# sohmandal/classpose

Measured on AMD Instinct MI355X. Metric: wsi_tiles_per_sec, higher is better.
Workload: dtype bf16; 1 GPU; configs[1]: synthetic 10000x10000 WSI (1936 tiles), tile 256 / overlap 32, conic 7 classes, ViT-L ClassTransformer depth 24 random-init, batch 32 sub-tiles = 8 WSI tiles/step, every step a distinct batch of the rank's shard (tiles sharded k % n_gpus, at most 256 distinct batches resident, longer runs wrap) streamed pinned host -> hipMemcpyAsync inside the timed region (the reader decodes ahead int; slide=10000, tile=256, overlap=32, batch_subtiles=32, distinct_batches=145, records_gathered=2048, decode_ahead_batches_at_t0=4, device_resident_batches_at_t0=1

## Files before the change

classpose_amd/_lib.py:

```python
from __future__ import annotations

import ctypes as C
import os
import subprocess

_HERE = os.path.dirname(os.path.abspath(__file__))
LIB_PATH = os.path.join(_HERE, "libclasspose_hip.so")
DEBUG_LIB_PATH = os.path.join(_HERE, "libclasspose_hip_debug.so")
CSRC = os.path.join(_HERE, "csrc")

ABI_VERSION = 3
DT_BF16, DT_F16, DT_F32 = 0, 1, 2
DTYPE_CODE = {"bf16": DT_BF16, "fp16": DT_F16, "fp32": DT_F32}
PROF_KINDS = ("fc1", "attention", "qkv", "proj", "fc2", "patch_embed", "neck_head")
FC1_KERNEL_NAME = "k_gemm4w<GELU + folded LayerNorm, one wave per SIMD> = void k_gemm4w<1, 0, false>(Gemm4wArgs)"


class CpxTiling(C.Structure):
    _fields_ = [("H", C.c_int), ("W", C.c_int), ("ypad1", C.c_int), ("xpad1", C.c_int),
                ("Ly", C.c_int), ("Lx", C.c_int), ("ny", C.c_int), ("nx", C.c_int),
                ("bsize", C.c_int), ("augment", C.c_int),
                ("ystart", C.c_int * 16), ("xstart", C.c_int * 16)]


# ... 128 lines not shown
    "cpx_stain_samples_workspace_bytes": (_sz, [_i, C.c_longlong]),
    "cpx_stain_samples": (_i, [_p, _p, _p, _i, C.c_longlong, _p, _d, _p, C.c_longlong, _p, _p, _p, _p, _sz, _p]),
    "cpx_he_stain_u8": (_i, [_p, _i, _i, _i, _p, _p, _p, _p, _p]),
    "cpx_warp_affine_pool_stain_u8": (_i, [_p, _p, _p, _p, _i, C.c_longlong, _p, _p, _i, _p, _p, _i, _p, _p, _p, _i, _i, _i, _p, _p,
                                           _p, _p]),
    "cpx_find_contours_ccomp_host": (_i, [_p, _i, _i, _p, _i, _p, _p, _p, _i]),
    "cpx_polygonize_workspace_bytes": (_sz, [_i, _i, _i, _i]),
    "cpx_polygonize_device": (_i, [_p, _p, _p, _i, _i, _i, _i, _d, _p, _p, _i, _p, _p, _p, _p]),
    "cpx_polygonize_host": (_i, [_p, _i, _i, _p, _i, _d, _d, _d, _p, _i, _p]),
    "cpx_dedup_pairs_workspace_bytes": (_sz, [_i, _i, _i]),
    "cpx_dedup_pairs": (_i, [_p, _i, _d, _d, _d, _i, _i, _d, _p, C.c_longlong, _p, _p, _sz, _p]),
    "cpx_write_geojson": (_i, [C.c_char_p, C.c_char_p, _p, C.c_int64, _p, _p, _p, _p, C.c_int64, _p, _i, _d, _d, _i]),
}
_PRIVATE = {
    "cpx_gemm_set_variant": (None, [_i]),
    "cpx_attention_set_variant": (None, [_i]),
    "cpx_gemm_set_nt": (None, [_i]),
    "cpx_follow_set_early_exit": (None, [_i]),
    "cpx_follow_set_lds_window": (None, [_i]),
    "cpx_gemm_set_reverse": (None, [_i]),
    "cpx_attention_set_xcd_order": (None, [_i]),
    "cpx_gemm_set_big": (None, [_i]),
    "cpx_gemm_set_persistent": (None, [_i]),
    "cpx_gemm_set_persistent_qkv": (None, [_i]),
    "cpx_postproc_set_fused": (None, [_i]),
    "cpx_gemm_set_direct": (None, [_i]),
    "cpx_gemm4w": (_i, [_p, _p, _i, _i, _i, _p, _p, _i, _p]),
    "cpx_gemm4w_set_variant": (None, [_i]),
    "cpx_gemm_set_4w": (None, [_i]),
    "cpx_net_set_mlp_parts": (None, [_i]),
    "cpx_gemm_set_balanced": (None, [_i]),
    "cpx_gemm_set_l2_block": (None, [_i]),
    "cpx_gemm_ln_dt": (_i, [_i, _p, _p, _i, _i, _i, _i, _p, _p, _p, _i, _p, _p, _p, _p]),
    "cpx_row_stats_dt": (_i, [_i, _p, _i, _p, _p]),
    "cpx_im2col3_f32_debug": (_i, [_p, _i, _p, _p]),
    "cpx_unet_head_layout": (_i, [C.POINTER(CpxConvOp), _i, _i, _i, C.POINTER(_sz), C.POINTER(_i)]),
}

_lib = None


class CpxError(RuntimeError):
    pass


def build(force: bool = False) -> str:
    if force:
# ... 98 lines not shown
```

classpose_amd/csrc/cpx_gemm.hip:

```cpp
#include "cpx_internal.h"
#include <type_traits>

typedef __attribute__((ext_vector_type(8))) __bf16 bf16x8;
typedef __attribute__((ext_vector_type(8))) _Float16 f16x8;
typedef __attribute__((ext_vector_type(4))) float f32x4;

#define BM 128
#define BN 128
#define BK 64
#define GEMM_THREADS 256
#define TILE_BYTES (128 * 128)
#define STAGE_BYTES (2 * TILE_BYTES)

template <bool NT_POSSIBLE, bool WT_POSSIBLE = false>
__device__ __forceinline__ void st16(void *p, uint4 v, bool nt, bool wt = false) {
    if (WT_POSSIBLE && wt) {
        typedef unsigned u32x4_t __attribute__((ext_vector_type(4)));
        u32x4_t w = {v.x, v.y, v.z, v.w};
        if (NT_POSSIBLE && nt) asm volatile("global_store_dwordx4 %0, %1, off sc1 nt" ::"v"(p), "v"(w) : "memory");
        else asm volatile("global_store_dwordx4 %0, %1, off sc1" ::"v"(p), "v"(w) : "memory");
    } else if (NT_POSSIBLE && nt) {
        typedef unsigned u32x4_t __attribute__((ext_vector_type(4)));
        u32x4_t w = {v.x, v.y, v.z, v.w};
        __builtin_nontemporal_store(w, reinterpret_cast<u32x4_t *>(p));
    } else {
        *reinterpret_cast<uint4 *>(p) = v;
    }
}
struct GemmArgs {
    const unsigned short *A;
    const unsigned short *W;
    int M, N, K;
    const float *bias;
    const void *aux;
    void *out;
    int ld_out;
    int tiles_n, n_blocks;
    int l2_block;
    int rev_m;
    int nt_out;
    const float *ln_stats;
    const float *ln_colsum;
    float *stats_out;
// ... 248 lines not shown
__device__ __forceinline__ void g2_read_x(u32x4 (&fx)[4][2], unsigned b0, unsigned b1) {
    fx[0][0] = lds_read128<HM * G2_HALF + 0 * 2048>(b0); fx[0][1] = lds_read128<HM * G2_HALF + 0 * 2048>(b1);
    fx[1][0] = lds_read128<HM * G2_HALF + 1 * 2048>(b0); fx[1][1] = lds_read128<HM * G2_HALF + 1 * 2048>(b1);
    fx[2][0] = lds_read128<HM * G2_HALF + 2 * 2048>(b0); fx[2][1] = lds_read128<HM * G2_HALF + 2 * 2048>(b1);
    fx[3][0] = lds_read128<HM * G2_HALF + 3 * 2048>(b0); fx[3][1] = lds_read128<HM * G2_HALF + 3 * 2048>(b1);
}
template <int HN>
__device__ __forceinline__ void g2_read_w(u32x4 (&fw)[2][2], unsigned b0, unsigned b1) {
    fw[0][0] = lds_read128<(2 + HN) * G2_HALF + 0 * 2048>(b0); fw[0][1] = lds_read128<(2 + HN) * G2_HALF + 0 * 2048>(b1);
    fw[1][0] = lds_read128<(2 + HN) * G2_HALF + 1 * 2048>(b0); fw[1][1] = lds_read128<(2 + HN) * G2_HALF + 1 * 2048>(b1);
}
template <bool F16, bool FIRST = false>
__device__ __forceinline__ void g2_mma(f32x4 (&acc)[4][2], const u32x4 (&fx)[4][2], const u32x4 (&fw)[2][2]) {
    __builtin_amdgcn_s_setprio(1);
#pragma unroll
    for (int ks = 0; ks < 2; ++ks)
#pragma unroll
        for (int mb = 0; mb < 4; ++mb)
#pragma unroll
            for (int nb = 0; nb < 2; ++nb)
                acc[mb][nb] = mfma16v<F16>(fw[nb][ks], fx[mb][ks], (FIRST && ks == 0) ? (f32x4){0.f, 0.f, 0.f, 0.f} : acc[mb][nb]);
    __builtin_amdgcn_s_setprio(0);
}
#define G2_BAR() __builtin_amdgcn_s_barrier()
#define G2_LGKM0() do { asm volatile("s_waitcnt lgkmcnt(0)" ::: "memory"); __builtin_amdgcn_sched_barrier(0); } while (0)

#define G2F_LN 1
#define G2F_STATS 2
#define G2F_BAL 64
#define G2F_DIRECT 32
template <int EPI, bool F16, int FLAGS>
__global__ void __launch_bounds__(G2_THREADS, 2) k_gemm256(GemmArgs g) {
    constexpr bool LN_IN = (FLAGS & G2F_LN) != 0 && EPI != CPX_EPI_RESID_BF16 && EPI != CPX_EPI_POS_BF16;
    constexpr bool STATS = (FLAGS & G2F_STATS) != 0 && (EPI == CPX_EPI_RESID_BF16 || EPI == CPX_EPI_POS_BF16);
    extern __shared__ __attribute__((aligned(16))) char smem[];
    const int tid = threadIdx.x, lane = tid & 63;
    const int wave = __builtin_amdgcn_readfirstlane(tid >> 6);
    const int wm = wave >> 2, wn = wave & 3;
    const int fr = lane & 15, fq = lane >> 4;
    int bid = blockIdx.x;
    {
        const int nxcd = 8, q = g.n_blocks / nxcd, r = g.n_blocks % nxcd, x = bid % nxcd;
        bid = (x < r ? x * (q + 1) : r * (q + 1) + (x - r) * q) + bid / nxcd;
    }
    int tile_m, tile_n;
    {
// ... 226 lines not shown
                if (c16 == 16)
                    *reinterpret_cast<float2 *>(g.stats_out + ((size_t)(m0 + ml) * LN_SLOTS + tile_n) * 2) = make_float2(sm, sq);
            }
        }
    }
}


#define G2P_STG_OFF G2_BUF
#define G2P_TAIL G2_LN_OFF
#define G2P_LDS_BYTES (G2_LN_OFF + 4096)
template <int EPI, bool F16, int FLAGS>
__global__ void __launch_bounds__(G2_THREADS, 2) k_gemm256p(GemmArgs g) {
    constexpr bool LN_IN = (FLAGS & G2F_LN) != 0 && EPI != CPX_EPI_RESID_BF16;
    constexpr bool STATS = (FLAGS & G2F_STATS) != 0 && EPI == CPX_EPI_RESID_BF16;
    extern __shared__ __attribute__((aligned(16))) char smem[];
    const int wave = __builtin_amdgcn_readfirstlane((int)threadIdx.x >> 6);
    const int wm = wave >> 2, wn = wave & 3;
    const int K = g.K, nk = K / 64, nblk = g.n_blocks, tiles_m = g.n_blocks / g.tiles_n;
    auto coords = [&](int v, int &m0_, int &n0_, int &tn_) {
        const int nxcd = 8, q = nblk / nxcd, r = nblk % nxcd, x = v % nxcd;
        int bid = (x < r ? x * (q + 1) : r * (q + 1) + (x - r) * q) + v / nxcd;
        int tile_m, tile_n;
        if (EPI == CPX_EPI_QKV_BF16 && g.l2_block == 3) {
            const int x = v & 7, slot = (v >> 3) & 31, i = v >> 8, rx = tiles_m >> 3, full = rx >> 4;
            int rg, cg;
            if (i < 6 * full) {
                const int rnd = i / 6, j = i - rnd * 6;
                rg = 2 * rnd + (j < 4 ? j >> 1 : j - 4); cg = j < 4 ? j & 1 : 2;
            } else {
                const int j = i - 6 * full;
                rg = 2 * full; cg = j < 2 ? j : 2;
            }
            tile_m = x * rx + rg * 8 + (slot >> 2);
            tile_n = cg * 4 + (slot & 3);
        } else if (g.l2_block && (tiles_m & 7) == 0 && (g.tiles_n & 3) == 0) {
            const int grp = bid >> 5, w_ = bid & 31, cgn = g.tiles_n >> 2, rgn = tiles_m >> 3;
            const int rg = g.l2_block == 2 ? grp % rgn : grp / cgn, cg = g.l2_block == 2 ? grp / rgn : grp - rg * cgn;
            tile_m = rg * 8 + (w_ >> 2);
            tile_n = cg * 4 + (w_ & 3);
        } else {
            tile_m = bid / g.tiles_n;
            tile_n = bid - tile_m * g.tiles_n;
        }
        if (g.rev_m) tile_m = tiles_m - 1 - tile_m;
        m0_ = tile_m * 256; n0_ = tile_n * 256; tn_ = tile_n;
    };
    char *sdst = smem + wave * 1024;
    const __amdgpu_buffer_rsrc_t rsrcX = __builtin_amdgcn_make_buffer_rsrc((void *)g.A, 0, 0x7FFFFFFF, 0x00020000);
    const __amdgpu_buffer_rsrc_t rsrcW = __builtin_amdgcn_make_buffer_rsrc((void *)g.W, 0, 0x7FFFFFFF, 0x00020000);
    const unsigned k64b = (unsigned)K * 128u, k128b = (unsigned)K * 256u;
    auto stage_at = [&](unsigned voff, unsigned sX, unsigned sW, int which, int t) {
        const unsigned so = (which < 2 ? sX : sW) + (which & 1) * k128b + (unsigned)t * 128u;
        char *d = sdst + (t & 1) * G2_BUF + which * G2_HALF;
        if (which < 2) {
            __builtin_amdgcn_raw_ptr_buffer_load_lds(rsrcX, (__attribute__((address_space(3))) void *)d, 16, voff, so, 0, 0);
            __builtin_amdgcn_raw_ptr_buffer_load_lds(rsrcX, (__attribute__((address_space(3))) void *)(d + 8192), 16, voff, so + k64b, 0, 0);
        } else {
            __builtin_amdgcn_raw_ptr_buffer_load_lds(rsrcW, (__attribute__((address_space(3))) void *)d, 16, voff, so, 0, 0);
            __builtin_amdgcn_raw_ptr_buffer_load_lds(rsrcW, (__attribute__((address_space(3))) void *)(d + 8192), 16, voff, so + k64b, 0, 0);
        }
    };
    const unsigned lds0 = (unsigned)(size_t)(__attribute__((address_space(3))) char *)smem;
    int v = blockIdx.x, m0, n0, tile_n;
    coords(v, m0, n0, tile_n);
    bool prefetched = false;
    for (;;) {
        const int vn = v + (int)gridDim.x;
        const bool has_next = vn < nblk;
        int m0n = 0, n0n = 0, tile_nn = 0;
        if (has_next) coords(vn, m0n, n0n, tile_nn);
        int tid = threadIdx.x;
        asm volatile("" : "+v"(tid));
        const int lane = tid & 63, fr = lane & 15, fq = lane >> 4, c16 = tid & 31;
        const int srow = tid >> 3, kc = (tid & 7) ^ (srow & 7);
        unsigned xb[2][2], wb[2][2];
#pragma unroll
        for (int ks = 0; ks < 2; ++ks) {
            const unsigned sw = (unsigned)(((ks * 4 + fq) ^ (fr & 7)) << 4);
            xb[0][ks] = lds0 + (wm * 64 + fr) * 128 + sw;
            wb[0][ks] = lds0 + (wn * 32 + fr) * 128 + sw;
            xb[1][ks] = xb[0][ks] + G2_BUF;
            wb[1][ks] = wb[0][ks] + G2_BUF;
        }
        const unsigned voff = ((unsigned)srow * (unsigned)K + (unsigned)kc * 8u) * 2u;
        const unsigned sX = (unsigned)m0 * (unsigned)K * 2u, sW = (unsigned)n0 * (unsigned)K * 2u;
        auto stage = [&](int which, int t) { stage_at(voff, sX, sW, which, t); };
        float4 st_a = make_float4(0.f, 0.f, 0.f, 0.f), st_b = st_a;
        float bias_v = 0.f, csum_v = 0.f;
        if (tid < 256) {
            if (LN_IN) {
                st_a = *reinterpret_cast<const float4 *>(g.ln_stats + (size_t)(m0 + tid) * 8);
                st_b = *reinterpret_cast<const float4 *>(g.ln_stats + (size_t)(m0 + tid) * 8 + 4);
            }
        } else {
            if (g.bias) bias_v = g.bias[n0 + tid - 256];
            if (LN_IN) csum_v = g.ln_colsum[n0 + tid - 256];
        }
        auto park_tile_vectors = [&]() {
            if (tid < 256) {
                if (LN_IN) {
                    const float inv_k = 1.0f / K;
                    const float sum = (st_a.x + st_a.z) + (st_b.x + st_b.z), sq = (st_a.y + st_a.w) + (st_b.y + st_b.w);
                    const float mean = sum * inv_k;
                    const float rstd = rsqrtf(fmaxf(sq * inv_k - mean * mean, 0.f) + 1e-6f);
                    *reinterpret_cast<float2 *>(smem + G2P_TAIL + tid * 8) = make_float2(rstd, -mean * rstd);
                }
            } else {
                *reinterpret_cast<float *>(smem + G2P_TAIL + 2048 + (tid - 256) * 4) = bias_v;
                *reinterpret_cast<float *>(smem + G2P_TAIL + 3072 + (tid - 256) * 4) = csum_v;
            }
        };
        constexpr bool BAL = (FLAGS & G2F_BAL) != 0;
        if (prefetched) {
            park_tile_vectors();
            if (nk > 1) { stage(0, 1); stage(3, 1); if constexpr (BAL) stage(2, 1); }
        } else {
            stage(0, 0); stage(2, 0); stage(3, 0); stage(1, 0);
            if (nk > 1) { stage(0, 1); stage(3, 1); if constexpr (BAL) stage(2, 1); }
            park_tile_vectors();
        }
        asm volatile("s_waitcnt lgkmcnt(0)" ::: "memory");
        if constexpr (BAL) asm volatile("s_waitcnt vmcnt(6)" ::: "memory");
        else if (nk > 1) asm volatile("s_waitcnt vmcnt(4)" ::: "memory");
        else asm volatile("s_waitcnt vmcnt(0)" ::: "memory");
        G2_BAR();
        f32x4 acc[2][2][4][2];
        u32x4 fx[4][2], fw[2][2], fw2[2][2];
        if constexpr (BAL) g2_read_w<0>(fw, wb[0][0], wb[0][1]);
// ... 62 lines not shown
        if constexpr (BAL) {
            G2_TILE_BAL(0, 0, true, 0, fw, fw2)
            G2_TILE_BAL(1, 1, false, 2, fw2, fw)
            for (int t = 2; t + 2 < nk; t += 2) {
                G2_TILE_BAL(t, 0, false, 2, fw, fw2)
                G2_TILE_BAL(t + 1, 1, false, 2, fw2, fw)
            }
            G2_TILE_BAL(nk - 2, 0, false, 3, fw, fw2)
            G2_TILE_BAL(nk - 1, 1, false, 4, fw2, fw)
        } else {
        G2_TILE_PLAIN(0, 0, true, -1)
        G2_TILE_PLAIN(1, 1, false, -1)
        for (int t = 2; t < nk; t += 2) {
            G2_TILE_PLAIN(t, 0, false, -1)
            G2_TILE_PLAIN(t + 1, 1, false, -1)
        }
        }
#undef G2_TILE_BAL
#undef G2_VM
#undef G2_TILE_PLAIN
        if (wm == 0) G2_BAR();
        __builtin_amdgcn_sched_barrier(0);

        const bool vt_tile = (EPI == CPX_EPI_QKV_BF16) && n0 >= 2048;
        bool next_issued = false;
        const unsigned sXn = (unsigned)m0n * (unsigned)K * 2u, sWn = (unsigned)n0n * (unsigned)K * 2u;
        auto prefetch_next = [&]() {
            stage_at(voff, sXn, sWn, 0, 0); stage_at(voff, sXn, sWn, 2, 0); stage_at(voff, sXn, sWn, 3, 0); stage_at(voff, sXn, sWn, 1, 0);
            next_issued = true;
        };
        if (vt_tile) {
#pragma unroll
            for (int hm = 0; hm < 2; ++hm)
#pragma unroll
                for (int hn = 0; hn < 2; ++hn)
#pragma unroll
                    for (int mb = 0; mb < 4; ++mb)
#pragma unroll
                        for (int nb = 0; nb < 2; ++nb) {
                            const int ml = hm * 128 + wm * 64 + mb * 16 + fr;
                            const int nl = hn * 128 + wn * 32 + nb * 16 + fq * 4;
                            f32x4 vv = acc[hm][hn][mb][nb];
                            const float4 b = *reinterpret_cast<const float4 *>(smem + G2P_TAIL + 2048 + nl * 4);
                            if constexpr (LN_IN) {
                                const float4 cs = *reinterpret_cast<const float4 *>(smem + G2P_TAIL + 3072 + nl * 4);
                                const float2 pr = *reinterpret_cast<const float2 *>(smem + G2P_TAIL + ml * 8);
                                vv[0] = fmaf(vv[0], pr.x, fmaf(pr.y, cs.x, b.x)); vv[1] = fmaf(vv[1], pr.x, fmaf(pr.y, cs.y, b.y));
                                vv[2] = fmaf(vv[2], pr.x, fmaf(pr.y, cs.z, b.z)); vv[3] = fmaf(vv[3], pr.x, fmaf(pr.y, cs.w, b.w));
                            } else {
                                vv[0] += b.x; vv[1] += b.y; vv[2] += b.z; vv[3] += b.w;
                            }
                            const unsigned p01 = pack2<F16>(vv[0], vv[1]), p23 = pack2<F16>(vv[2], vv[3]);
                            *reinterpret_cast<unsigned short *>(smem + (nl + 0) * G2_EPI_LD + ml * 2) = (unsigned short)p01;
                            *reinterpret_cast<unsigned short *>(smem + (nl + 1) * G2_EPI_LD + ml * 2) = (unsigned short)(p01 >> 16);
                            *reinterpret_cast<unsigned short *>(smem + (nl + 2) * G2_EPI_LD + ml * 2) = (unsigned short)p23;
                            *reinterpret_cast<unsigned short *>(smem + (nl + 3) * G2_EPI_LD + ml * 2) = (unsigned short)(p23 >> 16);
                        }
            asm volatile("s_waitcnt lgkmcnt(0)" ::: "memory");
            G2_BAR();
            unsigned short *vT = (unsigned short *)g.aux;
            const size_t s_ = (size_t)(m0 >> 10), t0 = (size_t)(m0 & 1023);
#pragma unroll 4
            for (int it = 0; it < 16; ++it) {
                const int row = it * 16 + (tid >> 5);
                const int c = n0 - 2048 + row;
                uint4 vv = *reinterpret_cast<const uint4 *>(smem + row * G2_EPI_LD + c16 * 16);
                st16<EPI == CPX_EPI_QKV_BF16, EPI == CPX_EPI_QKV_BF16>(vT + ((s_ * 16 + (c >> 6)) * 64 + (c & 63)) * 1024 + t0 + c16 * 8, vv, (g.nt_out & 4) != 0, (g.nt_out & 16) != 0);
            }
            asm volatile("s_waitcnt lgkmcnt(0)" ::: "memory");
            G2_BAR();
        } else if constexpr (EPI != CPX_EPI_RESID_BF16 && (FLAGS & G2F_DIRECT) != 0) {
            if (has_next) prefetch_next();
            const __amdgpu_buffer_rsrc_t rsrcO = __builtin_amdgcn_make_buffer_rsrc((void *)g.out, 0, 0x7FFFFFFF, 0x00020000);
            const unsigned ldb = (unsigned)g.ld_out * 2u;
            const unsigned ovoff = (unsigned)(wm * 64 + fr) * ldb + (unsigned)(wn * 32 + ((fq & 1) << 4) + ((fq >> 1) << 3)) * 2u;
            const unsigned so0 = (unsigned)m0 * ldb + (unsigned)n0 * 2u;
#pragma unroll
            for (int hm = 0; hm < 2; ++hm) {
                float ln_rs[4], ln_nm[4];
                if constexpr (LN_IN) {
#pragma unroll
                    for (int mb = 0; mb < 4; ++mb) {
                        const float2 pr = *reinterpret_cast<const float2 *>(smem + G2P_TAIL + (hm * 128 + wm * 64 + mb * 16 + fr) * 8);
                        ln_rs[mb] = pr.x; ln_nm[mb] = pr.y;
                    }
                }
#pragma unroll
                for (int hn = 0; hn < 2; ++hn) {
                    float4 b[2], cs[2];
#pragma unroll
                    for (int nb = 0; nb < 2; ++nb) {
                        const int nl = hn * 128 + wn * 32 + nb * 16 + fq * 4;
                        b[nb] = *reinterpret_cast<const float4 *>(smem + G2P_TAIL + 2048 + nl * 4);
                        cs[nb] = make_float4(0.f, 0.f, 0.f, 0.f);
// ... 11 lines not shown
                                vv[2] = fmaf(vv[2], rs, fmaf(nm, cs[nb].z, b[nb].z)); vv[3] = fmaf(vv[3], rs, fmaf(nm, cs[nb].w, b[nb].w));
                            } else {
                                vv[0] += b[nb].x; vv[1] += b[nb].y; vv[2] += b[nb].z; vv[3] += b[nb].w;
                            }
                            if constexpr (EPI == CPX_EPI_GELU_BF16) {
#pragma unroll
                                for (int r = 0; r < 4; ++r) vv[r] = gelu_erf(vv[r]);
                            } else if constexpr (EPI == CPX_EPI_RELU_BF16) {
#pragma unroll
                                for (int r = 0; r < 4; ++r) vv[r] = fmaxf(vv[r], 0.f);
                            }
                            pk[nb][0] = pack2<F16>(vv[0], vv[1]);
                            pk[nb][1] = pack2<F16>(vv[2], vv[3]);
                        }
                        const auto r0 = __builtin_amdgcn_permlane16_swap(pk[0][0], pk[1][0], false, false);
                        const auto r1 = __builtin_amdgcn_permlane16_swap(pk[0][1], pk[1][1], false, false);
                        const u32x4 o = {r0[0], r1[0], r0[1], r1[1]};
                        __builtin_amdgcn_raw_buffer_store_b128(o, rsrcO, ovoff, so0 + (unsigned)(hm * 128 + mb * 16) * ldb + (unsigned)hn * 256u, 0);
                    }
                }
            }
            G2_BAR();
        } else {
            if constexpr (EPI != CPX_EPI_RESID_BF16) {
                if (has_next) prefetch_next();
            }
            char *stg = smem + G2P_STG_OFF;
#pragma unroll
            for (int hm = 0; hm < 2; ++hm) {
                uint4 rres[8];
                if constexpr (EPI == CPX_EPI_RESID_BF16) {
#pragma unroll
                    for (int it = 0; it < 8; ++it)
                        rres[it] = *reinterpret_cast<const uint4 *>((const unsigned short *)g.aux +
                                                                    (size_t)(m0 + hm * 128 + it * 16 + (tid >> 5)) * g.ld_out + n0 + c16 * 8);
                }
                float ln_rs[4], ln_nm[4];
                if constexpr (LN_IN) {
#pragma unroll
                    for (int mb = 0; mb < 4; ++mb) {
                        const float2 pr = *reinterpret_cast<const float2 *>(smem + G2P_TAIL + (hm * 128 + wm * 64 + mb * 16 + fr) * 8);
                        ln_rs[mb] = pr.x; ln_nm[mb] = pr.y;
                    }
                }
#pragma unroll
                for (int hn = 0; hn < 2; ++hn)
#pragma unroll
                    for (int nb = 0; nb < 2; ++nb) {
                        const int nl = hn * 128 + wn * 32 + nb * 16 + fq * 4;
                        const float4 b = *reinterpret_cast<const float4 *>(smem + G2P_TAIL + 2048 + nl * 4);
                        float4 cs = make_float4(0.f, 0.f, 0.f, 0.f);
                        if constexpr (LN_IN) cs = *reinterpret_cast<const float4 *>(smem + G2P_TAIL + 3072 + nl * 4);
#pragma unroll
                        for (int mb = 0; mb < 4; ++mb) {
                            const int mlh = wm * 64 + mb * 16 + fr;
                            f32x4 vv = acc[hm][hn][mb][nb];
                            if constexpr (LN_IN) {
                                const float nm = ln_nm[mb], rs = ln_rs[mb];
                                vv[0] = fmaf(vv[0], rs, fmaf(nm, cs.x, b.x)); vv[1] = fmaf(vv[1], rs, fmaf(nm, cs.y, b.y));
                                vv[2] = fmaf(vv[2], rs, fmaf(nm, cs.z, b.z)); vv[3] = fmaf(vv[3], rs, fmaf(nm, cs.w, b.w));
                            } else {
                                vv[0] += b.x; vv[1] += b.y; vv[2] += b.z; vv[3] += b.w;
                            }
                            if constexpr (EPI == CPX_EPI_GELU_BF16) {
#pragma unroll
                                for (int r = 0; r < 4; ++r) vv[r] = gelu_erf(vv[r]);
                            } else if constexpr (EPI == CPX_EPI_RELU_BF16) {
#pragma unroll
                                for (int r = 0; r < 4; ++r) vv[r] = fmaxf(vv[r], 0.f);
                            }
                            uint2 o;
                            o.x = pack2<F16>(vv[0], vv[1]);
                            o.y = pack2<F16>(vv[2], vv[3]);
                            *reinterpret_cast<uint2 *>(stg + mlh * G2_EPI_LD + nl * 2) = o;
                        }
                    }
                asm volatile("s_waitcnt lgkmcnt(0)" ::: "memory");
                G2_BAR();
#pragma unroll
                for (int it = 0; it < 8; ++it) {
                    const int mlh = it * 16 + (tid >> 5);
                    uint4 vv = *reinterpret_cast<const uint4 *>(stg + mlh * G2_EPI_LD + c16 * 16);
                    const int ml = hm * 128 + mlh;
                    const size_t go = (size_t)(m0 + ml) * g.ld_out + n0 + c16 * 8;
                    if constexpr (EPI == CPX_EPI_RESID_BF16) {
                        const uint4 rr = rres[it];
                        unsigned a[4] = {vv.x, vv.y, vv.z, vv.w}, b[4] = {rr.x, rr.y, rr.z, rr.w};
#pragma unroll
                        for (int i = 0; i < 4; ++i) {
                            float lo = from_half<F16>(a[i] & 0xFFFF) + from_half<F16>(b[i] & 0xFFFF);
                            float hi = from_half<F16>(a[i] >> 16) + from_half<F16>(b[i] >> 16);
                            a[i] = pack2<F16>(lo, hi);
                        }
                        vv = make_uint4(a[0], a[1], a[2], a[3]);
                    }
                    st16<EPI == CPX_EPI_QKV_BF16, EPI == CPX_EPI_RESID_BF16 || EPI == CPX_EPI_QKV_BF16>((unsigned short *)g.out + go, vv, (g.nt_out & (n0 < 1024 ? 1 : 2)) != 0,
                                                                                        (g.nt_out & (EPI == CPX_EPI_QKV_BF16 ? 16 : 8)) != 0);
                    if constexpr (STATS) {
                        unsigned a[4] = {vv.x, vv.y, vv.z, vv.w};
                        float sm = 0.f, sq = 0.f;
#pragma unroll
                        for (int i = 0; i < 4; ++i) {
                            const float lo = from_half<F16>(a[i] & 0xFFFF), hi = from_half<F16>(a[i] >> 16);
                            sm += lo + hi; sq += lo * lo + hi * hi;
                        }
                        sm = half_wave_sum(sm); sq = half_wave_sum(sq);
                        if (c16 == 16)
                            *reinterpret_cast<float2 *>(g.stats_out + ((size_t)(m0 + ml) * LN_SLOTS + tile_n) * 2) = make_float2(sm, sq);
                    }
                }
                asm volatile("s_waitcnt lgkmcnt(0)" ::: "memory");
                G2_BAR();
            }
        }
        if (!has_next) break;
        prefetched = next_issued;
        v = vn; m0 = m0n; n0 = n0n; tile_n = tile_nn;
    }
}

CPX_SWITCH(g_gemm_persist, 1);
CPX_SWITCH(g_gemm_variant, 1);
CPX_SWITCH(g_gemm_l2, 1);
CPX_SWITCH(g_gemm_persist_qkv, 1);
CPX_SWITCH(g_gemm_rev, 0);
CPX_SWITCH(g_gemm_big, 1);
CPX_SWITCH(g_gemm_bal, 1);
CPX_SWITCH(g_gemm_direct, 1);
CPX_SWITCH(g_gemm_nt, 15);
CPX_SWITCH(g_gemm_4w, 1);
#ifdef CPX_DEBUG
extern "C" void cpx_gemm_set_persistent(int on) { g_gemm_persist = on; }
extern "C" void cpx_gemm_set_variant(int glds) { g_gemm_variant = glds; }
extern "C" void cpx_gemm_set_persistent_qkv(int on) { g_gemm_persist_qkv = on; }
extern "C" void cpx_gemm_set_l2_block(int on) { g_gemm_l2 = on; }
extern "C" void cpx_gemm_set_reverse(int on) { g_gemm_rev = on; }
extern "C" void cpx_gemm_set_big(int on) { g_gemm_big = on; }
extern "C" void cpx_gemm_set_direct(int on) { g_gemm_direct = on; }
extern "C" void cpx_gemm_set_balanced(int on) { g_gemm_bal = on; }
extern "C" void cpx_gemm_set_4w(int on) { g_gemm_4w = on; }
extern "C" void cpx_gemm_set_nt(int on) { g_gemm_nt = on; }
#endif

template <int EPI, bool F16, int FLAGS>
static void launch_gemm256_flags(const GemmArgs &a, hipStream_t s) {
    const bool qkv_balanced = EPI == CPX_EPI_QKV_BF16 && g_gemm_persist_qkv && (a.n_blocks / a.tiles_n) % 64 == 0 && a.tiles_n == 12;
    const bool fits32 = (size_t)a.M * (size_t)a.K * 2 < ((size_t)1 << 31) && (size_t)a.N * (size_t)a.K * 2 < ((size_t)1 << 31);
    if (g_gemm_persist && fits32 && (EPI != CPX_EPI_QKV_BF16 || qkv_balanced)) {
        static CpxOncePerDevice once_p;
        static int n_cu = 0;
        once_p([] {
            (void)hipFuncSetAttribute((const void *)k_gemm256p<EPI, F16, FLAGS>, hipFuncAttributeMaxDynamicSharedMemorySize, G2P_LDS_BYTES);
            int dev = 0, cus = 256;
            (void)hipGetDevice(&dev);
            (void)hipDeviceGetAttribute(&cus, hipDeviceAttributeMultiprocessorCount, dev);
            n_cu = cus > 0 ? cus : 256;
        });
        if (EPI == CPX_EPI_QKV_BF16) {
            if (n_cu == 256) {
                GemmArgs b = a;
                b.l2_block = 3;
                hipLaunchKernelGGL((k_gemm256p<EPI, F16, FLAGS>), dim3(256), dim3(G2_THREADS), G2P_LDS_BYTES, s, b);
                return;
            }
        } else {
            const int grid = a.n_blocks < n_cu ? a.n_blocks : n_cu;
            hipLaunchKernelGGL((k_gemm256p<EPI, F16, FLAGS>), dim3(grid), dim3(G2_THREADS), G2P_LDS_BYTES, s, a);
            return;
        }
    }
    static CpxOncePerDevice once;
    once([] { (void)hipFuncSetAttribute((const void *)k_gemm256<EPI, F16, FLAGS>, hipFuncAttributeMaxDynamicSharedMemorySize, G2_LDS_BYTES); });
    hipLaunchKernelGGL((k_gemm256<EPI, F16, FLAGS>), dim3(a.n_blocks), dim3(G2_THREADS), G2_LDS_BYTES, s, a);
}

template <int EPI, bool F16>
static bool launch_gemm256(const GemmArgs &a0, hipStream_t s) {
    if constexpr (EPI == CPX_EPI_F32) return false;
    else {
        if (!g_gemm_big || a0.M % 256 || a0.N % 256 || a0.K < 128) return false;
        if ((a0.K / 64) % 2 && EPI != CPX_EPI_POS_BF16) return false;
        if ((a0.M / 256) * (a0.N / 256) < 256) return false;
        GemmArgs a = a0;
        a.tiles_n = a.N / 256; a.n_blocks = (a.M / 256) * (a.N / 256);
        constexpr bool PRODUCER = EPI == CPX_EPI_RESID_BF16 || EPI == CPX_EPI_POS_BF16;
        constexpr int F1 = PRODUCER ? G2F_STATS : G2F_LN;
        const bool f1 = PRODUCER ? a.stats_out != nullptr : a.ln_stats != nullptr;
        if constexpr (EPI == CPX_EPI_POS_BF16) {
            static CpxOncePerDevice once_pos;
            once_pos([] {
                (void)hipFuncSetAttribute((const void *)k_gemm256<EPI, F16, 0>, hipFuncAttributeMaxDynamicSharedMemorySize, G2_LDS_BYTES);
                (void)hipFuncSetAttribute((const void *)k_gemm256<EPI, F16, G2F_STATS>, hipFuncAttributeMaxDynamicSharedMemorySize, G2_LDS_BYTES);
// ... 183 lines not shown
```

include/classpose_hip_debug.h:

```cpp
#ifndef CLASSPOSE_HIP_DEBUG_H
#define CLASSPOSE_HIP_DEBUG_H
#ifdef __cplusplus
extern "C" {
#endif
void cpx_gemm_set_variant(int glds);
void cpx_gemm_set_big(int on);
void cpx_gemm_set_persistent(int on);
void cpx_gemm_set_persistent_qkv(int on);
void cpx_gemm_set_l2_block(int on);
void cpx_gemm_set_reverse(int on);
void cpx_gemm_set_direct(int mode);
void cpx_gemm_set_balanced(int on);
int cpx_gemm4w(const void *A, const void *W, int M, int N, int K, const float *bias, void *out, int ld_out, void *stream);
void cpx_gemm_set_4w(int on);
void cpx_gemm4w_set_variant(int v);
void cpx_net_set_mlp_parts(int on);
void cpx_attention_set_xcd_order(int on);
void cpx_attention_set_variant(int v);
void cpx_postproc_set_fused(int on);
void cpx_gemm_set_nt(int on);
void cpx_follow_set_early_exit(int on);
void cpx_follow_set_lds_window(int on);
int cpx_row_stats_dt(int dtype, const void *x, int rows, float *stats, void *stream);
int cpx_gemm_ln_dt(int dtype, const void *A, const void *Wt, int M, int N, int K, int epilogue,
                   const float *bias, const void *aux, void *out, int ld_out,
                   const float *ln_stats, const float *ln_colsum, float *stats_out, void *stream);
int cpx_im2col3_f32_debug(const float *x, int n_subtiles, float *out, void *stream);
struct cpx_conv_op;
int cpx_unet_head_layout(const struct cpx_conv_op *ops, int n_ops, int n_subtiles, int dtype, size_t *dst_off, int *ld);
#ifdef __cplusplus
}
// ... 3 lines not shown
```

Baseline: 371.9 tiles/s.

## Restructure persistent GEMM epilogue: swap V-transpose operands, prefetch residual, drop QKV remap

For QKV tiles that write the transposed V, the persistent GEMM now swaps the A and W operands, so the accumulator already lands in transposed order. This removes the separate scatter-transpose epilogue path. The residual epilogue issues its residual loads before the next-tile prefetch, waits on explicit vmcnt/lgkmcnt counters, and uses inline-asm LDS reads for the row and column scale factors. It also drops the special l2_block==3 QKV tile mapping and its toggle, so the QKV GEMM uses the generic grid and L2 grouping, and it adds an s_nop after write-through stores. The hand-tuned waitcnt values are fragile and could be wrong, and dropping the custom QKV mapping may hurt L2 reuse.

```diff
diff --git a/classpose_amd/_lib.py b/classpose_amd/_lib.py
--- a/classpose_amd/_lib.py
+++ b/classpose_amd/_lib.py
@@ -174,7 +174,6 @@
     "cpx_attention_set_xcd_order": (None, [_i]),
     "cpx_gemm_set_big": (None, [_i]),
     "cpx_gemm_set_persistent": (None, [_i]),
-    "cpx_gemm_set_persistent_qkv": (None, [_i]),
     "cpx_postproc_set_fused": (None, [_i]),
     "cpx_gemm_set_direct": (None, [_i]),
     "cpx_gemm4w": (_i, [_p, _p, _i, _i, _i, _p, _p, _i, _p]),
diff --git a/classpose_amd/csrc/cpx_gemm.hip b/classpose_amd/csrc/cpx_gemm.hip
--- a/classpose_amd/csrc/cpx_gemm.hip
+++ b/classpose_amd/csrc/cpx_gemm.hip
@@ -1,5 +1,6 @@
 #include "cpx_internal.h"
 #include <type_traits>
+#include <utility>
 
 typedef __attribute__((ext_vector_type(8))) __bf16 bf16x8;
 typedef __attribute__((ext_vector_type(8))) _Float16 f16x8;
@@ -17,8 +18,8 @@
     if (WT_POSSIBLE && wt) {
         typedef unsigned u32x4_t __attribute__((ext_vector_type(4)));
         u32x4_t w = {v.x, v.y, v.z, v.w};
-        if (NT_POSSIBLE && nt) asm volatile("global_store_dwordx4 %0, %1, off sc1 nt" ::"v"(p), "v"(w) : "memory");
-        else asm volatile("global_store_dwordx4 %0, %1, off sc1" ::"v"(p), "v"(w) : "memory");
+        if (NT_POSSIBLE && nt) asm volatile("global_store_dwordx4 %0, %1, off sc1 nt\n\ts_nop 1" ::"v"(p), "v"(w) : "memory");
+        else asm volatile("global_store_dwordx4 %0, %1, off sc1\n\ts_nop 1" ::"v"(p), "v"(w) : "memory");
     } else if (NT_POSSIBLE && nt) {
         typedef unsigned u32x4_t __attribute__((ext_vector_type(4)));
         u32x4_t w = {v.x, v.y, v.z, v.w};
@@ -313,6 +314,44 @@
                 acc[mb][nb] = mfma16v<F16>(fw[nb][ks], fx[mb][ks], (FIRST && ks == 0) ? (f32x4){0.f, 0.f, 0.f, 0.f} : acc[mb][nb]);
     __builtin_amdgcn_s_setprio(0);
 }
+__device__ __forceinline__ void load128_unseen(u32x4 &r, unsigned voff, const void *sbase) {
+    asm volatile("global_load_dwordx4 %0, %1, %2" : "=v"(r) : "v"(voff), "s"(sbase) : "memory");
+}
+template <int N>
+__device__ __forceinline__ void wait_vmcnt_for(u32x4 &r) {
+    asm volatile("s_waitcnt vmcnt(%1)" : "+v"(r) : "n"(N) : "memory");
+}
+template <int N>
+__device__ __forceinline__ void wait_vmcnt(void) {
+    asm volatile("s_waitcnt vmcnt(%0)" : : "n"(N) : "memory");
+}
+__device__ __forceinline__ void arrived(u32x4 &r) {
+    __builtin_amdgcn_sched_barrier(0);
+    asm volatile("" : "+v"(r) : : "memory");
+}
+typedef __attribute__((ext_vector_type(2))) unsigned u32x2;
+template <int OFF>
+__device__ __forceinline__ float lds_read32f(unsigned addr) {
+    float v;
+    asm volatile("ds_read_b32 %0, %1 offset:%2" : "=v"(v) : "v"(addr), "n"(OFF) : "memory");
+    return v;
+}
+template <int OFF>
+__device__ __forceinline__ f32x4 lds_read128f(unsigned addr) {
+    f32x4 v;
+    asm volatile("ds_read_b128 %0, %1 offset:%2" : "=v"(v) : "v"(addr), "n"(OFF) : "memory");
+    return v;
+}
+template <int OFF>
+__device__ __forceinline__ void lds_write64(unsigned addr, u32x2 v) {
+    asm volatile("ds_write_b64 %0, %1 offset:%2" : : "v"(addr), "v"(v), "n"(OFF) : "memory");
+}
+template <int N>
+__device__ __forceinline__ void wait_lgkmcnt_for(u32x4 &r) {
+    asm volatile("s_waitcnt lgkmcnt(%1)" : "+v"(r) : "n"(N) : "memory");
+}
+template <int... I, class F>
+__device__ __forceinline__ void static_for(std::integer_sequence<int, I...>, F &&f) { (f(std::integral_constant<int, I>{}), ...); }
 #define G2_BAR() __builtin_amdgcn_s_barrier()
 #define G2_LGKM0() do { asm volatile("s_waitcnt lgkmcnt(0)" ::: "memory"); __builtin_amdgcn_sched_barrier(0); } while (0)
 
@@ -585,19 +624,7 @@
         const int nxcd = 8, q = nblk / nxcd, r = nblk % nxcd, x = v % nxcd;
         int bid = (x < r ? x * (q + 1) : r * (q + 1) + (x - r) * q) + v / nxcd;
         int tile_m, tile_n;
-        if (EPI == CPX_EPI_QKV_BF16 && g.l2_block == 3) {
-            const int x = v & 7, slot = (v >> 3) & 31, i = v >> 8, rx = tiles_m >> 3, full = rx >> 4;
-            int rg, cg;
-            if (i < 6 * full) {
-                const int rnd = i / 6, j = i - rnd * 6;
-                rg = 2 * rnd + (j < 4 ? j >> 1 : j - 4); cg = j < 4 ? j & 1 : 2;
-            } else {
-                const int j = i - 6 * full;
-                rg = 2 * full; cg = j < 2 ? j : 2;
-            }
-            tile_m = x * rx + rg * 8 + (slot >> 2);
-            tile_n = cg * 4 + (slot & 3);
-        } else if (g.l2_block && (tiles_m & 7) == 0 && (g.tiles_n & 3) == 0) {
+        if (g.l2_block && (tiles_m & 7) == 0 && (g.tiles_n & 3) == 0) {
             const int grp = bid >> 5, w_ = bid & 31, cgn = g.tiles_n >> 2, rgn = tiles_m >> 3;
             const int rg = g.l2_block == 2 ? grp % rgn : grp / cgn, cg = g.l2_block == 2 ? grp / rgn : grp - rg * cgn;
             tile_m = rg * 8 + (w_ >> 2);
@@ -610,10 +637,12 @@
         m0_ = tile_m * 256; n0_ = tile_n * 256; tn_ = tile_n;
     };
     char *sdst = smem + wave * 1024;
-    const __amdgpu_buffer_rsrc_t rsrcX = __builtin_amdgcn_make_buffer_rsrc((void *)g.A, 0, 0x7FFFFFFF, 0x00020000);
-    const __amdgpu_buffer_rsrc_t rsrcW = __builtin_amdgcn_make_buffer_rsrc((void *)g.W, 0, 0x7FFFFFFF, 0x00020000);
+    auto operand_rsrc = [&](bool weights) {
+        return __builtin_amdgcn_make_buffer_rsrc((void *)(weights ? g.W : g.A), 0, 0x7FFFFFFF, 0x00020000);
+    };
+    auto is_vt = [&](int n0_) { return EPI == CPX_EPI_QKV_BF16 && n0_ >= 2048; };
     const unsigned k64b = (unsigned)K * 128u, k128b = (unsigned)K * 256u;
-    auto stage_at = [&](unsigned voff, unsigned sX, unsigned sW, int which, int t) {
+    auto stage_at = [&](__amdgpu_buffer_rsrc_t rsrcX, __amdgpu_buffer_rsrc_t rsrcW, unsigned voff, unsigned sX, unsigned sW, int which, int t) {
         const unsigned so = (which < 2 ? sX : sW) + (which & 1) * k128b + (unsigned)t * 128u;
         char *d = sdst + (t & 1) * G2_BUF + which * G2_HALF;
         if (which < 2) {
@@ -635,7 +664,7 @@
         if (has_next) coords(vn, m0n, n0n, tile_nn);
         int tid = threadIdx.x;
         asm volatile("" : "+v"(tid));
-        const int lane = tid & 63, fr = lane & 15, fq = lane >> 4, c16 = tid & 31;
+        const int lane = tid & 63, fr = lane & 15, fq = lane >> 4;
         const int srow = tid >> 3, kc = (tid & 7) ^ (srow & 7);
         unsigned xb[2][2], wb[2][2];
 #pragma unroll
@@ -647,8 +676,10 @@
             wb[1][ks] = wb[0][ks] + G2_BUF;
         }
         const unsigned voff = ((unsigned)srow * (unsigned)K + (unsigned)kc * 8u) * 2u;
-        const unsigned sX = (unsigned)m0 * (unsigned)K * 2u, sW = (unsigned)n0 * (unsigned)K * 2u;
-        auto stage = [&](int which, int t) { stage_at(voff, sX, sW, which, t); };
+        const bool vt_tile = is_vt(n0);
+        const __amdgpu_buffer_rsrc_t rsrcX = operand_rsrc(vt_tile), rsrcW = operand_rsrc(!vt_tile);
+        const unsigned sX = (unsigned)(vt_tile ? n0 : m0) * (unsigned)K * 2u, sW = (unsigned)(vt_tile ? m0 : n0) * (unsigned)K * 2u;
+        auto stage = [&](int which, int t) { stage_at(rsrcX, rsrcW, voff, sX, sW, which, t); };
         float4 st_a = make_float4(0.f, 0.f, 0.f, 0.f), st_b = st_a;
         float bias_v = 0.f, csum_v = 0.f;
         if (tid < 256) {
@@ -667,7 +698,12 @@
                     const float sum = (st_a.x + st_a.z) + (st_b.x + st_b.z), sq = (st_a.y + st_a.w) + (st_b.y + st_b.w);
                     const float mean = sum * inv_k;
                     const float rstd = rsqrtf(fmaxf(sq * inv_k - mean * mean, 0.f) + 1e-6f);
-                    *reinterpret_cast<float2 *>(smem + G2P_TAIL + tid * 8) = make_float2(rstd, -mean * rstd);
+                    if (vt_tile) {
+                        *reinterpret_cast<float *>(smem + G2P_TAIL + tid * 4) = rstd;
+                        *reinterpret_cast<float *>(smem + G2P_TAIL + 1024 + tid * 4) = -mean * rstd;
+                    } else {
+                        *reinterpret_cast<float2 *>(smem + G2P_TAIL + tid * 8) = make_float2(rstd, -mean * rstd);
+                    }
                 }
             } else {
                 *reinterpret_cast<float *>(smem + G2P_TAIL + 2048 + (tid - 256) * 4) = bias_v;
@@ -776,54 +812,16 @@
         if (wm == 0) G2_BAR();
         __builtin_amdgcn_sched_barrier(0);
 
-        const bool vt_tile = (EPI == CPX_EPI_QKV_BF16) && n0 >= 2048;
         bool next_issued = false;
-        const unsigned sXn = (unsigned)m0n * (unsigned)K * 2u, sWn = (unsigned)n0n * (unsigned)K * 2u;
+        const bool vt_next = is_vt(n0n);
+        const __amdgpu_buffer_rsrc_t rsrcXn = operand_rsrc(vt_next), rsrcWn = operand_rsrc(!vt_next);
+        const unsigned sXn = (unsigned)(vt_next ? n0n : m0n) * (unsigned)K * 2u, sWn = (unsigned)(vt_next ? m0n : n0n) * (unsigned)K * 2u;
         auto prefetch_next = [&]() {
-            stage_at(voff, sXn, sWn, 0, 0); stage_at(voff, sXn, sWn, 2, 0); stage_at(voff, sXn, sWn, 3, 0); stage_at(voff, sXn, sWn, 1, 0);
+            stage_at(rsrcXn, rsrcWn, voff, sXn, sWn, 0, 0); stage_at(rsrcXn, rsrcWn, voff, sXn, sWn, 2, 0);
+            stage_at(rsrcXn, rsrcWn, voff, sXn, sWn, 3, 0); stage_at(rsrcXn, rsrcWn, voff, sXn, sWn, 1, 0);
             next_issued = true;
         };
-        if (vt_tile) {
-#pragma unroll
-            for (int hm = 0; hm < 2; ++hm)
-#pragma unroll
-                for (int hn = 0; hn < 2; ++hn)
-#pragma unroll
-                    for (int mb = 0; mb < 4; ++mb)
-#pragma unroll
-                        for (int nb = 0; nb < 2; ++nb) {
-                            const int ml = hm * 128 + wm * 64 + mb * 16 + fr;
-                            const int nl = hn * 128 + wn * 32 + nb * 16 + fq * 4;
-                            f32x4 vv = acc[hm][hn][mb][nb];
-                            const float4 b = *reinterpret_cast<const float4 *>(smem + G2P_TAIL + 2048 + nl * 4);
-                            if constexpr (LN_IN) {
-                                const float4 cs = *reinterpret_cast<const float4 *>(smem + G2P_TAIL + 3072 + nl * 4);
-                                const float2 pr = *reinterpret_cast<const float2 *>(smem + G2P_TAIL + ml * 8);
-                                vv[0] = fmaf(vv[0], pr.x, fmaf(pr.y, cs.x, b.x)); vv[1] = fmaf(vv[1], pr.x, fmaf(pr.y, cs.y, b.y));
-                                vv[2] = fmaf(vv[2], pr.x, fmaf(pr.y, cs.z, b.z)); vv[3] = fmaf(vv[3], pr.x, fmaf(pr.y, cs.w, b.w));
-                            } else {
-                                vv[0] += b.x; vv[1] += b.y; vv[2] += b.z; vv[3] += b.w;
-                            }
-                            const unsigned p01 = pack2<F16>(vv[0], vv[1]), p23 = pack2<F16>(vv[2], vv[3]);
-                            *reinterpret_cast<unsigned short *>(smem + (nl + 0) * G2_EPI_LD + ml * 2) = (unsigned short)p01;
-                            *reinterpret_cast<unsigned short *>(smem + (nl + 1) * G2_EPI_LD + ml * 2) = (unsigned short)(p01 >> 16);
-                            *reinterpret_cast<unsigned short *>(smem + (nl + 2) * G2_EPI_LD + ml * 2) = (unsigned short)p23;
-                            *reinterpret_cast<unsigned short *>(smem + (nl + 3) * G2_EPI_LD + ml * 2) = (unsigned short)(p23 >> 16);
-                        }
-            asm volatile("s_waitcnt lgkmcnt(0)" ::: "memory");
-            G2_BAR();
-            unsigned short *vT = (unsigned short *)g.aux;
-            const size_t s_ = (size_t)(m0 >> 10), t0 = (size_t)(m0 & 1023);
-#pragma unroll 4
-            for (int it = 0; it < 16; ++it) {
-                const int row = it * 16 + (tid >> 5);
-                const int c = n0 - 2048 + row;
-                uint4 vv = *reinterpret_cast<const uint4 *>(smem + row * G2_EPI_LD + c16 * 16);
-                st16<EPI == CPX_EPI_QKV_BF16, EPI == CPX_EPI_QKV_BF16>(vT + ((s_ * 16 + (c >> 6)) * 64 + (c & 63)) * 1024 + t0 + c16 * 8, vv, (g.nt_out & 4) != 0, (g.nt_out & 16) != 0);
-            }
-            asm volatile("s_waitcnt lgkmcnt(0)" ::: "memory");
-            G2_BAR();
-        } else if constexpr (EPI != CPX_EPI_RESID_BF16 && (FLAGS & G2F_DIRECT) != 0) {
+        if constexpr (EPI != CPX_EPI_RESID_BF16 && (FLAGS & G2F_DIRECT) != 0) {
             if (has_next) prefetch_next();
             const __amdgpu_buffer_rsrc_t rsrcO = __builtin_amdgcn_make_buffer_rsrc((void *)g.out, 0, 0x7FFFFFFF, 0x00020000);
             const unsigned ldb = (unsigned)g.ld_out * 2u;
@@ -881,45 +879,79 @@
             }
             G2_BAR();
         } else {
-            if constexpr (EPI != CPX_EPI_RESID_BF16) {
+            constexpr bool RESID = EPI == CPX_EPI_RESID_BF16;
+            auto staged_rows = [&](auto vt_tag) {
+                constexpr bool VT = decltype(vt_tag)::value;
+                int tid = threadIdx.x;
+                asm volatile("" : "+v"(tid));
+                const int fr = tid & 15, fq = (tid & 63) >> 4, c16 = tid & 31;
+                const unsigned row_addr = lds0 + G2P_TAIL + (VT ? 2048u + (unsigned)(wm * 64 + fr) * 4u : (unsigned)(wm * 64 + fr) * 8u);
+                const unsigned col_addr = lds0 + G2P_TAIL + (unsigned)(wn * 32 + fq * 4) * 4u;
+                const unsigned stw_addr = lds0 + G2P_STG_OFF + (unsigned)(wm * 64 + fr) * G2_EPI_LD + (unsigned)(wn * 32 + fq * 4) * 2u;
+                const unsigned str_addr = lds0 + G2P_STG_OFF + (unsigned)(tid >> 5) * G2_EPI_LD + (unsigned)c16 * 16u;
+                u32x4 rres[8];
+                unsigned rvoff = 0;
+                const char *rbase = nullptr;
+                const size_t r16 = (size_t)g.ld_out * 32;
+                if constexpr (RESID) {
+                    rvoff = ((unsigned)(tid >> 5) * (unsigned)g.ld_out + (unsigned)c16 * 8u) * 2u;
+                    rbase = (const char *)g.aux + ((size_t)m0 * g.ld_out + n0) * 2;
+#pragma unroll
+                    for (int it = 0; it < 8; ++it) load128_unseen(rres[it], rvoff, rbase + it * r16);
+                }
                 if (has_next) prefetch_next();
-            }
-            char *stg = smem + G2P_STG_OFF;
-#pragma unroll
-            for (int hm = 0; hm < 2; ++hm) {
-                uint4 rres[8];
-                if constexpr (EPI == CPX_EPI_RESID_BF16) {
-#pragma unroll
-                    for (int it = 0; it < 8; ++it)
-                        rres[it] = *reinterpret_cast<const uint4 *>((const unsigned short *)g.aux +
-                                                                    (size_t)(m0 + hm * 128 + it * 16 + (tid >> 5)) * g.ld_out + n0 + c16 * 8);
-                }
-                float ln_rs[4], ln_nm[4];
-                if constexpr (LN_IN) {
-#pragma unroll
-                    for (int mb = 0; mb < 4; ++mb) {
-                        const float2 pr = *reinterpret_cast<const float2 *>(smem + G2P_TAIL + (hm * 128 + wm * 64 + mb * 16 + fr) * 8);
-                        ln_rs[mb] = pr.x; ln_nm[mb] = pr.y;
+                auto half = [&](auto hm_tag) {
+                    constexpr int hm = decltype(hm_tag)::value;
+                    float row_a[4] = {0.f, 0.f, 0.f, 0.f}, row_b[4] = {0.f, 0.f, 0.f, 0.f};
+                    if constexpr (VT || LN_IN) {
+                        static_for(std::make_integer_sequence<int, 4>{}, [&](auto mb_tag) {
+                            constexpr int mb = decltype(mb_tag)::value, r = hm * 128 + mb * 16;
+                            if constexpr (VT) {
+                                row_a[mb] = lds_read32f<r * 4>(row_addr);
+                                if constexpr (LN_IN) row_b[mb] = lds_read32f<1024 + r * 4>(row_addr);
+                            } else {
+                                row_a[mb] = lds_read32f<r * 8>(row_addr);
+                                row_b[mb] = lds_read32f<r * 8 + 4>(row_addr);
+                            }
+                        });
                     }
-                }
-#pragma unroll
-                for (int hn = 0; hn < 2; ++hn)
-#pragma unroll
-                    for (int nb = 0; nb < 2; ++nb) {
-                        const int nl = hn * 128 + wn * 32 + nb * 16 + fq * 4;
-                        const float4 b = *reinterpret_cast<const float4 *>(smem + G2P_TAIL + 2048 + nl * 4);
-                        float4 cs = make_float4(0.f, 0.f, 0.f, 0.f);
-                        if constexpr (LN_IN) cs = *reinterpret_cast<const float4 *>(smem + G2P_TAIL + 3072 + nl * 4);
-#pragma unroll
-                        for (int mb = 0; mb < 4; ++mb) {
-                            const int mlh = wm * 64 + mb * 16 + fr;
+                    f32x4 colb[2] = {{0.f, 0.f, 0.f, 0.f}, {0.f, 0.f, 0.f, 0.f}}, colc[2] = {{0.f, 0.f, 0.f, 0.f}, {0.f, 0.f, 0.f, 0.f}};
+                    auto read_cols = [&](auto g_tag) {
+                        constexpr int gi = decltype(g_tag)::value, o = ((gi >> 1) * 128 + (gi & 1) * 16) * 4, p = gi & 1;
+                        if constexpr (VT) {
+                            if constexpr (LN_IN) { colb[p] = lds_read128f<o>(col_addr); colc[p] = lds_read128f<1024 + o>(col_addr); }
+                        } else {
+                            colb[p] = lds_read128f<2048 + o>(col_addr);
+                            if constexpr (LN_IN) colc[p] = lds_read128f<3072 + o>(col_addr);
+                        }
+                    };
+                    read_cols(std::integral_constant<int, 0>{});
+                    static_for(std::make_integer_sequence<int, 4>{}, [&](auto g_tag) {
+                        constexpr int gi = decltype(g_tag)::value, hn = gi >> 1, nb = gi & 1, p = gi & 1;
+                        asm volatile("s_waitcnt lgkmcnt(0)" : "+v"(colb[p]), "+v"(colc[p]) : : "memory");
+                        if constexpr (gi == 0) {
+#pragma unroll
+                            for (int mb = 0; mb < 4; ++mb) asm volatile("" : "+v"(row_a[mb]), "+v"(row_b[mb]));
+                        }
+                        if constexpr (gi < 3) read_cols(std::integral_constant<int, gi + 1>{});
+                        const f32x4 b = colb[p], cs = colc[p];
+                        static_for(std::make_integer_sequence<int, 4>{}, [&](auto mb_tag) {
+                            constexpr int mb = decltype(mb_tag)::value;
                             f32x4 vv = acc[hm][hn][mb][nb];
-                            if constexpr (LN_IN) {
-                                const float nm = ln_nm[mb], rs = ln_rs[mb];
-                                vv[0] = fmaf(vv[0], rs, fmaf(nm, cs.x, b.x)); vv[1] = fmaf(vv[1], rs, fmaf(nm, cs.y, b.y));
-                                vv[2] = fmaf(vv[2], rs, fmaf(nm, cs.z, b.z)); vv[3] = fmaf(vv[3], rs, fmaf(nm, cs.w, b.w));
+                            if constexpr (VT) {
+                                const float bc = row_a[mb], cc = row_b[mb];
+                                if constexpr (LN_IN) {
+                                    vv[0] = fmaf(vv[0], b[0], fmaf(cs[0], cc, bc)); vv[1] = fmaf(vv[1], b[1], fmaf(cs[1], cc, bc));
+                                    vv[2] = fmaf(vv[2], b[2], fmaf(cs[2], cc, bc)); vv[3] = fmaf(vv[3], b[3], fmaf(cs[3], cc, bc));
+                                } else {
+                                    vv[0] += bc; vv[1] += bc; vv[2] += bc; vv[3] += bc;
+                                }
+                            } else if constexpr (LN_IN) {
+                                const float nm = row_b[mb], rs = row_a[mb];
+                                vv[0] = fmaf(vv[0], rs, fmaf(nm, cs[0], b[0])); vv[1] = fmaf(vv[1], rs, fmaf(nm, cs[1], b[1]));
+                                vv[2] = fmaf(vv[2], rs, fmaf(nm, cs[2], b[2])); vv[3] = fmaf(vv[3], rs, fmaf(nm, cs[3], b[3]));
                             } else {
-                                vv[0] += b.x; vv[1] += b.y; vv[2] += b.z; vv[3] += b.w;
+                                vv[0] += b[0]; vv[1] += b[1]; vv[2] += b[2]; vv[3] += b[3];
                             }
                             if constexpr (EPI == CPX_EPI_GELU_BF16) {
 #pragma unroll
@@ -928,48 +960,73 @@
 #pragma unroll
                                 for (int r = 0; r < 4; ++r) vv[r] = fmaxf(vv[r], 0.f);
                             }
-                            uint2 o;
-                            o.x = pack2<F16>(vv[0], vv[1]);
-                            o.y = pack2<F16>(vv[2], vv[3]);
-                            *reinterpret_cast<uint2 *>(stg + mlh * G2_EPI_LD + nl * 2) = o;
+                            const u32x2 o = {pack2<F16>(vv[0], vv[1]), pack2<F16>(vv[2], vv[3])};
+                            lds_write64<mb * 16 * G2_EPI_LD + hn * 256 + nb * 32>(stw_addr, o);
+                        });
+                    });
+                    asm volatile("s_waitcnt lgkmcnt(0)" ::: "memory");
+                    G2_BAR();
+                    u32x4 srow[8];
+                    static_for(std::make_integer_sequence<int, 8>{}, [&](auto it_tag) {
+                        constexpr int it = decltype(it_tag)::value;
+                        srow[it] = lds_read128<it * 16 * G2_EPI_LD>(str_addr);
+                    });
+                    static_for(std::make_integer_sequence<int, 8>{}, [&](auto it_tag) {
+                        constexpr int it = decltype(it_tag)::value;
+                        const int ml = hm * 128 + it * 16 + (tid >> 5);
+                        wait_lgkmcnt_for<7 - it>(srow[it]);
+                        uint4 vv = make_uint4(srow[it][0], srow[it][1], srow[it][2], srow[it][3]);
+                        if constexpr (RESID) {
+                            if constexpr (hm == 0) {
+                                if (has_next) wait_vmcnt<15 + it>();
+                                else wait_vmcnt<7 + it>();
+                                arrived(rres[it]);
+                            } else {
+                                wait_vmcnt_for<14 - it>(rres[it]);
+                            }
+                            const u32x4 rr = rres[it];
+                            unsigned a[4] = {vv.x, vv.y, vv.z, vv.w}, b[4] = {rr[0], rr[1], rr[2], rr[3]};
+#pragma unroll
+                            for (int i = 0; i < 4; ++i) {
+                                float lo = from_half<F16>(a[i] & 0xFFFF) + from_half<F16>(b[i] & 0xFFFF);
+                                float hi = from_half<F16>(a[i] >> 16) + from_half<F16>(b[i] >> 16);
+                                a[i] = pack2<F16>(lo, hi);
+                            }
+                            vv = make_uint4(a[0], a[1], a[2], a[3]);
                         }
-                    }
-                asm volatile("s_waitcnt lgkmcnt(0)" ::: "memory");
-                G2_BAR();
-#pragma unroll
-                for (int it = 0; it < 8; ++it) {
-                    const int mlh = it * 16 + (tid >> 5);
-                    uint4 vv = *reinterpret_cast<const uint4 *>(stg + mlh * G2_EPI_LD + c16 * 16);
-                    const int ml = hm * 128 + mlh;
-                    const size_t go = (size_t)(m0 + ml) * g.ld_out + n0 + c16 * 8;
-                    if constexpr (EPI == CPX_EPI_RESID_BF16) {
-                        const uint4 rr = rres[it];
-                        unsigned a[4] = {vv.x, vv.y, vv.z, vv.w}, b[4] = {rr.x, rr.y, rr.z, rr.w};
-#pragma unroll
-                        for (int i = 0; i < 4; ++i) {
-                            float lo = from_half<F16>(a[i] & 0xFFFF) + from_half<F16>(b[i] & 0xFFFF);
-                            float hi = from_half<F16>(a[i] >> 16) + from_half<F16>(b[i] >> 16);
-                            a[i] = pack2<F16>(lo, hi);
+                        if constexpr (VT) {
+                            unsigned short *vT = (unsigned short *)g.aux;
+                            const size_t c = (size_t)(m0 >> 10) * 1024 + (size_t)(n0 - 2048 + ml);
+                            st16<true, true>(vT + c * 1024 + (size_t)(m0 & 1023) + c16 * 8, vv, (g.nt_out & 4) != 0, (g.nt_out & 16) != 0);
+                        } else {
+                            const size_t go = (size_t)(m0 + ml) * g.ld_out + n0 + c16 * 8;
+                            st16<EPI == CPX_EPI_QKV_BF16, EPI == CPX_EPI_RESID_BF16 || EPI == CPX_EPI_QKV_BF16>((unsigned short *)g.out + go, vv, (g.nt_out & (n0 < 1024 ? 1 : 2)) != 0,
+                                                                                                (g.nt_out & (EPI == CPX_EPI_QKV_BF16 ? 16 : 8)) != 0);
                         }
-                        vv = make_uint4(a[0], a[1], a[2], a[3]);
-                    }
-                    st16<EPI == CPX_EPI_QKV_BF16, EPI == CPX_EPI_RESID_BF16 || EPI == CPX_EPI_QKV_BF16>((unsigned short *)g.out + go, vv, (g.nt_out & (n0 < 1024 ? 1 : 2)) != 0,
-                                                                                        (g.nt_out & (EPI == CPX_EPI_QKV_BF16 ? 16 : 8)) != 0);
-                    if constexpr (STATS) {
-                        unsigned a[4] = {vv.x, vv.y, vv.z, vv.w};
-                        float sm = 0.f, sq = 0.f;
-#pragma unroll
-                        for (int i = 0; i < 4; ++i) {
-                            const float lo = from_half<F16>(a[i] & 0xFFFF), hi = from_half<F16>(a[i] >> 16);
-                            sm += lo + hi; sq += lo * lo + hi * hi;
+                        if constexpr (RESID && hm == 0) load128_unseen(rres[it], rvoff, rbase + (8 + it) * r16);
+                        if constexpr (STATS) {
+                            unsigned a[4] = {vv.x, vv.y, vv.z, vv.w};
+                            float sm = 0.f, sq = 0.f;
+#pragma unroll
+                            for (int i = 0; i < 4; ++i) {
+                                const float lo = from_half<F16>(a[i] & 0xFFFF), hi = from_half<F16>(a[i] >> 16);
+                                sm += lo + hi; sq += lo * lo + hi * hi;
+                            }
+                            sm = half_wave_sum(sm); sq = half_wave_sum(sq);
+                            if (c16 == 16)
+                                *reinterpret_cast<float2 *>(g.stats_out + ((size_t)(m0 + ml) * LN_SLOTS + tile_n) * 2) = make_float2(sm, sq);
                         }
-                        sm = half_wave_sum(sm); sq = half_wave_sum(sq);
-                        if (c16 == 16)
-                            *reinterpret_cast<float2 *>(g.stats_out + ((size_t)(m0 + ml) * LN_SLOTS + tile_n) * 2) = make_float2(sm, sq);
-                    }
-                }
-                asm volatile("s_waitcnt lgkmcnt(0)" ::: "memory");
-                G2_BAR();
+                    });
+                    G2_BAR();
+                };
+                half(std::integral_constant<int, 0>{});
+                half(std::integral_constant<int, 1>{});
+            };
+            if constexpr (EPI == CPX_EPI_QKV_BF16) {
+                if (vt_tile) staged_rows(std::true_type{});
+                else staged_rows(std::false_type{});
+            } else {
+                staged_rows(std::false_type{});
             }
         }
         if (!has_next) break;
@@ -981,7 +1038,6 @@
 CPX_SWITCH(g_gemm_persist, 1);
 CPX_SWITCH(g_gemm_variant, 1);
 CPX_SWITCH(g_gemm_l2, 1);
-CPX_SWITCH(g_gemm_persist_qkv, 1);
 CPX_SWITCH(g_gemm_rev, 0);
 CPX_SWITCH(g_gemm_big, 1);
 CPX_SWITCH(g_gemm_bal, 1);
@@ -991,7 +1047,6 @@
 #ifdef CPX_DEBUG
 extern "C" void cpx_gemm_set_persistent(int on) { g_gemm_persist = on; }
 extern "C" void cpx_gemm_set_variant(int glds) { g_gemm_variant = glds; }
-extern "C" void cpx_gemm_set_persistent_qkv(int on) { g_gemm_persist_qkv = on; }
 extern "C" void cpx_gemm_set_l2_block(int on) { g_gemm_l2 = on; }
 extern "C" void cpx_gemm_set_reverse(int on) { g_gemm_rev = on; }
 extern "C" void cpx_gemm_set_big(int on) { g_gemm_big = on; }
@@ -1003,9 +1058,9 @@
 
 template <int EPI, bool F16, int FLAGS>
 static void launch_gemm256_flags(const GemmArgs &a, hipStream_t s) {
-    const bool qkv_balanced = EPI == CPX_EPI_QKV_BF16 && g_gemm_persist_qkv && (a.n_blocks / a.tiles_n) % 64 == 0 && a.tiles_n == 12;
+    const bool qkv_ok = EPI != CPX_EPI_QKV_BF16 || ((a.n_blocks / a.tiles_n) % 64 == 0 && a.tiles_n == 12);
     const bool fits32 = (size_t)a.M * (size_t)a.K * 2 < ((size_t)1 << 31) && (size_t)a.N * (size_t)a.K * 2 < ((size_t)1 << 31);
-    if (g_gemm_persist && fits32 && (EPI != CPX_EPI_QKV_BF16 || qkv_balanced)) {
+    if (g_gemm_persist && fits32 && qkv_ok) {
         static CpxOncePerDevice once_p;
         static int n_cu = 0;
         once_p([] {
@@ -1015,18 +1070,9 @@
             (void)hipDeviceGetAttribute(&cus, hipDeviceAttributeMultiprocessorCount, dev);
             n_cu = cus > 0 ? cus : 256;
         });
-        if (EPI == CPX_EPI_QKV_BF16) {
-            if (n_cu == 256) {
-                GemmArgs b = a;
-                b.l2_block = 3;
-                hipLaunchKernelGGL((k_gemm256p<EPI, F16, FLAGS>), dim3(256), dim3(G2_THREADS), G2P_LDS_BYTES, s, b);
-                return;
-            }
-        } else {
-            const int grid = a.n_blocks < n_cu ? a.n_blocks : n_cu;
-            hipLaunchKernelGGL((k_gemm256p<EPI, F16, FLAGS>), dim3(grid), dim3(G2_THREADS), G2P_LDS_BYTES, s, a);
-            return;
-        }
+        const int grid = a.n_blocks < n_cu ? a.n_blocks : n_cu;
+        hipLaunchKernelGGL((k_gemm256p<EPI, F16, FLAGS>), dim3(grid), dim3(G2_THREADS), G2P_LDS_BYTES, s, a);
+        return;
     }
     static CpxOncePerDevice once;
     once([] { (void)hipFuncSetAttribute((const void *)k_gemm256<EPI, F16, FLAGS>, hipFuncAttributeMaxDynamicSharedMemorySize, G2_LDS_BYTES); });
diff --git a/include/classpose_hip_debug.h b/include/classpose_hip_debug.h
--- a/include/classpose_hip_debug.h
+++ b/include/classpose_hip_debug.h
@@ -6,7 +6,6 @@
 void cpx_gemm_set_variant(int glds);
 void cpx_gemm_set_big(int on);
 void cpx_gemm_set_persistent(int on);
-void cpx_gemm_set_persistent_qkv(int on);
 void cpx_gemm_set_l2_block(int on);
 void cpx_gemm_set_reverse(int on);
 void cpx_gemm_set_direct(int mode);
```

New measurement: 373.0 tiles/s (median of 6 runs). No clear change (+0.3%).
